# guangkun0818/speech2text

Measured on AMD Instinct MI355X. Metric: audio-seconds/sec (train step, zipformer pruned-RNN-T), higher is better.
Workload: dtype f32; 1 GPU; C3 zipformer pruned-RNN-T train step: chunk_size -1, 500 BPE, prune_range 5 (fbank+fwd+bwd+allreduce+ScaledAdam); accumulate_grad_batches=1, gemm_arith=bf16x2/3, per_gpu_batch=64, global_batch=64, labels_per_utt=50, parallelism=dp1

## Files before the change

include/s2t_mi355.h:

```cpp
#ifndef S2T_MI355_H_
#define S2T_MI355_H_

#ifdef __cplusplus
extern "C" {
#endif

int s2t_fbank_f32(const float* pcm, long pcm_stride, const long* num_samples, int batch,
                  const float* window400, const float* twiddle512, const int* mel_off,
                  const int* mel_k0, const float* mel_w, int nnz, int num_mel, float eps,
                  float scale_in, const float* cmvn_mean, const float* cmvn_istd, float* out,
                  int max_frames, long* out_frames, void* stream);

#define S2T_CTC_MAX_LABELS 1023
long s2t_ctc_workspace_floats(int B, int T, int Umax);
int s2t_ctc_loss_fwd_bwd(const float* logits, const long* targets, long tgt_stride,
                         const long* in_len, const long* tgt_len, int B, int T, int V, int Umax,
                         int blank, int zero_infinity, const float* grad_scale, float* workspace,
                         float* loss_per_utt, float* grad_logits, void* stream);

int s2t_fill_f32(float* p, long n, float v, void* stream);
int s2t_rnnt_row_exp(const float* x, long rows, int C, float* probs, float* rowmax, void* stream);
int s2t_rnnt_simple_pxpy(const float* am, const float* lm, const float* am_max,
                         const float* lm_max, const float* nrm, const long* symbols,
                         const long* boundary, int B, int S, int T, int C, int blank, float* px,
// ... 222 lines not shown
int s2t_specaug(float* feats, int B, int T, int F, const int* tspan, int nt, const int* fspan,
                int nf, void* stream);
int s2t_pad_rows(const float* packed, const long* offsets, int B, long Lmax, int D, float* out,
                 void* stream);

int s2t_linear_lt(int mode, const float* X, long ldx, const float* W, long ldw, const float* bias,
                  const float* C, long ldc, float beta, float* D, long ldd, int M, int N, int K,
                  void* workspace, long ws_bytes, void* stream);
int s2t_linear_lt_stats(int* plans, int* timed);
long s2t_linear_lt_own_calls(void);

int s2t_bypass_fwd(const float* orig, const float* src, const float* scale, long rows, int C,
                   float* out, void* stream);
int s2t_bypass_bwd(const float* orig, const float* src, const float* scale, const float* g,
                   long rows, int C, float* d_orig, float* d_src, float* d_scale, void* stream);
int s2t_bypass_bwd_acc(const float* orig, const float* src, const float* scale, const float* g,
                       const float* acc_in, long rows, int C, float* d_orig, float* d_src,
                       float* d_scale, void* stream);
int s2t_attn_delta_pairs(const float* W, const float* dW0, const float* dO1, const float* O1,
                         int dv1, const float* dO2, const float* O2, int dv2, int T, int B, int H,
                         float* delta, void* stream);
int s2t_bypass_fwd_mask(const float* orig, const float* src, const float* scale, const float* fm,
                        int B, long rows, int C, float* out, void* stream);
int s2t_bypass_bwd_mask(const float* orig, const float* src, const float* scale, const float* g,
                        const float* fm, int B, long rows, int C, float* d_orig, float* d_src,
                        float* d_scale, void* stream);
int s2t_downsample_fwd(const float* src, const float* w, int ds, int T, int B, int C, float* out,
                       void* stream);
int s2t_downsample_bwd(const float* src, const float* w, const float* g, int ds, int T, int B, int C,
                       float* d_src, float* dw, void* stream);
int s2t_downsample_fwd_bt(const float* src, const float* w, int ds, int T, int B, int C, float* out,
                          void* stream);
int s2t_downsample_bwd_bt(const float* src, const float* w, const float* g, int ds, int T, int B, int C,
                          float* d_src, float* dw, void* stream);
int s2t_bypass_up_fwd(const float* orig, const float* src, const float* scale, int up, int T, int B,
                      int C, float* out, void* stream);
int s2t_bypass_up_bwd(const float* orig, const float* src, const float* scale, const float* g, int up,
                      int T, int B, int C, float* d_orig, float* d_src, float* d_scale, void* stream);
typedef struct S2tCommit {
  const float* x;
  float* d;
  float* grad;
  float lo, hi;
  int limit;
  long n;
} S2tCommit;
int s2t_param_grad_commit_n(int n, const S2tCommit* items, void* stream);
int s2t_nonlin_gate_fwd(const float* u, int T, int B, int C, float* xs, void* stream);
int s2t_nonlin_out_fwd(const float* z, const float* u, int T, int B, int C, float* o, void* stream);
int s2t_nonlin_out_bwd(const float* g, const float* z, const float* u, int T, int B, int C, float* dz,
                       float* du, void* stream);
int s2t_nonlin_gate_bwd(const float* dxs, const float* u, int T, int B, int C, float* du,
                        void* stream);

int s2t_layernorm_fwd(const float* x, const float* y, float alpha, const float* gamma,
                      const float* beta, long rows, int C, float eps, float* xsum, float* out,
                      float* stats, void* stream);
typedef struct S2tLnFold {
  const float* partial;
  long rows;
  float* dgamma;
  float* dbeta;
} S2tLnFold;
long s2t_layernorm_bwd_partial_floats(long rows, int C);
int s2t_layernorm_bwd(const float* x, const float* stats, const float* gamma, const float* dy,
                      const float* resid, long rows, int C, float* dx, float* partial,
                      void* stream);
int s2t_layernorm_param_grad(int n, const S2tLnFold* items, int C, void* stream);
int s2t_silu_fwd(const float* h, long n, float* a, void* stream);
int s2t_silu_bwd(const float* h, const float* da, long n, float scale, float* dh, void* stream);
int s2t_dropout_add(const float* x, const float* y, long n, float alpha, float p,
                    unsigned long long seed, float* out, void* stream);
int s2t_silu_drop_fwd(const float* h, long n, float p, unsigned long long seed, float* a,
                      void* stream);
int s2t_silu_drop_bwd(const float* h, const float* da, long n, float scale, float p,
                      unsigned long long seed, float* dh, void* stream);
#define S2T_BN_PARTIALS 128
long s2t_bn_workspace_floats(int C);
int s2t_bn_silu_fwd(const float* x, const float* gamma, const float* beta, float eps,
                    float momentum, float* running_mean, float* running_var, long* num_batches,
                    long rows, int C, float* y, float* save_mean, float* save_rstd,
                    float* workspace, void* stream);
int s2t_bn_silu_apply(const float* x, const float* mean, const float* rstd, const float* gamma,
                      const float* beta, long rows, int C, float* y, void* stream);
int s2t_bn_silu_bwd(const float* x, const float* ds, const float* save_mean,
                    const float* save_rstd, const float* gamma, const float* beta, long rows, int C,
                    float* dx, float* dgamma, float* dbeta, float* workspace, void* stream);
int s2t_mhsa_fwd(const float* qkv, long ld, int qoff, int koff, int voff, const long* lens, int T,
                 int B, int H, int dh, float scale, float dropout_p, unsigned long seed, float* o,
                 long ldo, float* lse, void* stream);
int s2t_mhsa_bwd(const float* qkv, long ld, int qoff, int koff, int voff, const long* lens, int T,
                 int B, int H, int dh, float scale, float dropout_p, unsigned long seed,
                 const float* o, const float* d_o, long ldo, const float* lse, float* delta,
                 float* dqkv, void* stream);

long s2t_conv1_relu_workspace_floats(int C);
int s2t_conv1_relu_fwd(const float* x, const float* w, const float* bias, int B, int T, int F,
                       int C, float* out, void* stream);
int s2t_conv1_relu_wgrad(const float* x, const float* w, const float* bias, const float* d_out,
                         int B, int T, int F, int C, float* dw, float* db, float* workspace,
                         void* stream);

#define S2T_ADAM_MAX_GROUPS 8
typedef struct S2tAdamGroup {
  int chunk_hi;
  float lr, beta1, beta2, eps, weight_decay;
// ... 192 lines not shown
```

speech2text_amd/csrc/zip_glue.hip:

```cpp
#include "common.h"
#include "../../include/s2t_mi355.h"

namespace {

constexpr int RB = 64;

__global__ __launch_bounds__(256) void bypass_fwd_kernel(const float* __restrict__ orig,
                                                         const float* __restrict__ src,
                                                         const float* __restrict__ scale, long n4,
                                                         int C4, float* __restrict__ out) {
  const float4* o4 = reinterpret_cast<const float4*>(orig);
  const float4* s4 = reinterpret_cast<const float4*>(src);
  const float4* sc4 = reinterpret_cast<const float4*>(scale);
  float4* y4 = reinterpret_cast<float4*>(out);
  for (long i = (long)blockIdx.x * 256 + threadIdx.x; i < n4; i += (long)gridDim.x * 256) {
    const float4 a = o4[i], b = s4[i], k = sc4[i % C4];
    y4[i] = make_float4(fmaf(b.x - a.x, k.x, a.x), fmaf(b.y - a.y, k.y, a.y),
                        fmaf(b.z - a.z, k.z, a.z), fmaf(b.w - a.w, k.w, a.w));
  }
}

__global__ __launch_bounds__(256) void bypass_bwd_kernel(const float* __restrict__ orig,
                                                         const float* __restrict__ src,
                                                         const float* __restrict__ scale,
// ... 427 lines not shown
    const long t = tb / B;
    const float* row = u + tb * 3 * C;
    xs[((long)b * T + t) * C + c] = row[C + c] * tanhf(row[c]);
  }
}

__global__ __launch_bounds__(256) void nonlin_out_fwd_kernel(const float* __restrict__ z,
                                                             const float* __restrict__ u, int T,
                                                             int B, int C, float* __restrict__ o) {
  const long n = (long)T * B * C;
  for (long i = (long)blockIdx.x * 256 + threadIdx.x; i < n; i += (long)gridDim.x * 256) {
    const int c = (int)(i % C);
    const long tb = i / C;
    const int b = (int)(tb % B);
    const long t = tb / B;
    o[i] = z[((long)b * T + t) * C + c] * u[tb * 3 * C + 2 * C + c];
  }
}

__global__ __launch_bounds__(256) void nonlin_out_bwd_kernel(const float* __restrict__ g,
                                                             const float* __restrict__ z,
                                                             const float* __restrict__ u, int T,
                                                             int B, int C, float* __restrict__ dz,
                                                             float* __restrict__ du) {
  const long n = (long)T * B * C;
  for (long i = (long)blockIdx.x * 256 + threadIdx.x; i < n; i += (long)gridDim.x * 256) {
    const int c = (int)(i % C);
    const long tb = i / C;
    const int b = (int)(tb % B);
    const long t = tb / B;
    const long zi = ((long)b * T + t) * C + c;
    const float gv = g[i];
    dz[zi] = gv * u[tb * 3 * C + 2 * C + c];
    du[tb * 3 * C + 2 * C + c] = gv * z[zi];
  }
}

__global__ __launch_bounds__(256) void nonlin_gate_bwd_kernel(const float* __restrict__ dxs,
                                                              const float* __restrict__ u, int T,
                                                              int B, int C,
                                                              float* __restrict__ du) {
  const long n = (long)T * B * C;
  for (long i = (long)blockIdx.x * 256 + threadIdx.x; i < n; i += (long)gridDim.x * 256) {
    const int c = (int)(i % C);
    const long tb = i / C;
    const int b = (int)(tb % B);
    const long t = tb / B;
    const float d = dxs[((long)b * T + t) * C + c];
    const float* row = u + tb * 3 * C;
    const float th = tanhf(row[c]);
    du[tb * 3 * C + c] = d * row[C + c] * (1.f - th * th);
    du[tb * 3 * C + C + c] = d * th;
  }
}

inline unsigned grid1(long n) {
  long g = (n + 255) / 256;
  return (unsigned)(g > 4096 ? 4096 : (g < 1 ? 1 : g));
}

}

extern "C" int s2t_bypass_fwd(const float* orig, const float* src, const float* scale, long rows,
                              int C, float* out, void* stream) {
  if (rows <= 0) return 0;
  if (C <= 0 || (C & 3)) return -1;
  const long n4 = rows * C / 4;
  hipLaunchKernelGGL(bypass_fwd_kernel, dim3(grid1(n4)), dim3(256), 0, (hipStream_t)stream, orig,
                     src, scale, n4, C / 4, out);
  S2T_CHECK_LAUNCH();
  return 0;
}

extern "C" int s2t_bypass_bwd(const float* orig, const float* src, const float* scale,
                              const float* g, long rows, int C, float* d_orig, float* d_src,
                              float* d_scale, void* stream) {
  if (rows <= 0) return 0;
  if (C <= 0) return -1;
  hipLaunchKernelGGL(bypass_bwd_kernel, dim3((unsigned)((rows + RB - 1) / RB)), dim3(256), 0,
                     (hipStream_t)stream, orig, src, scale, g, rows, C, d_orig, d_src, d_scale);
  S2T_CHECK_LAUNCH();
  return 0;
}

extern "C" int s2t_bypass_bwd_acc(const float* orig, const float* src, const float* scale,
                                  const float* g, const float* acc_in, long rows, int C,
                                  float* d_orig, float* d_src, float* d_scale, void* stream) {
  if (rows <= 0) return 0;
  if (C <= 0 || !acc_in) return -1;
  hipLaunchKernelGGL(bypass_bwd_acc_kernel, dim3((unsigned)((rows + RB - 1) / RB)), dim3(256), 0,
                     (hipStream_t)stream, orig, src, scale, g, acc_in, rows, C, d_orig, d_src,
                     d_scale);
  S2T_CHECK_LAUNCH();
  return 0;
}

extern "C" int s2t_attn_delta_pairs(const float* W, const float* dW0, const float* dO1,
                                    const float* O1, int dv1, const float* dO2, const float* O2,
                                    int dv2, int T, int B, int H, float* delta, void* stream) {
  if (T <= 0 || B <= 0 || H <= 0) return 0;
  if (dv1 > 64 || dv2 > 64 || dv1 < 0 || dv2 < 0) return -1;
  const long rows = (long)H * B * T;
  hipLaunchKernelGGL(attn_delta_pairs_kernel, dim3((unsigned)((rows + 3) / 4)), dim3(256), 0,
                     (hipStream_t)stream, W, dW0, dO1, O1, dv1, dO2, O2, dv2, T, B, H, delta);
  S2T_CHECK_LAUNCH();
  return 0;
// ... 127 lines not shown
    nb = (nb + m - 1) / m * m;
#define BUP4(UP, IU)                                                                                          \
  hipLaunchKernelGGL((bypass_up_bwd4_kernel<UP, IU>), dim3((unsigned)nb), dim3(256), 0, (hipStream_t)stream,  \
                     reinterpret_cast<const float4*>(orig), reinterpret_cast<const float4*>(src),             \
                     reinterpret_cast<const float4*>(scale), reinterpret_cast<const float4*>(g), T, F, C4, n, \
                     reinterpret_cast<float4*>(d_orig), reinterpret_cast<float4*>(d_src), d_scale)
    if (up == 2) BUP4(2, 4);
    else if (up == 4) BUP4(4, 2);
    else BUP4(8, 1);
#undef BUP4
    S2T_CHECK_LAUNCH();
    return 0;
  }
  hipLaunchKernelGGL(bypass_up_bwd_kernel, dim3(Ts, (B + 15) / 16), dim3(256), 0,
                     (hipStream_t)stream, orig, src, scale, g, up, T, B, C, d_orig, d_src, d_scale);
  S2T_CHECK_LAUNCH();
  return 0;
}

extern "C" int s2t_nonlin_gate_fwd(const float* u, int T, int B, int C, float* xs, void* stream) {
  if (T <= 0 || B <= 0 || C <= 0) return 0;
  hipLaunchKernelGGL(nonlin_gate_fwd_kernel, dim3(grid1((long)T * B * C)), dim3(256), 0,
                     (hipStream_t)stream, u, T, B, C, xs);
  S2T_CHECK_LAUNCH();
  return 0;
}

extern "C" int s2t_nonlin_out_fwd(const float* z, const float* u, int T, int B, int C, float* o,
                                  void* stream) {
  if (T <= 0 || B <= 0 || C <= 0) return 0;
  hipLaunchKernelGGL(nonlin_out_fwd_kernel, dim3(grid1((long)T * B * C)), dim3(256), 0,
                     (hipStream_t)stream, z, u, T, B, C, o);
  S2T_CHECK_LAUNCH();
  return 0;
}

extern "C" int s2t_nonlin_out_bwd(const float* g, const float* z, const float* u, int T, int B,
                                  int C, float* dz, float* du, void* stream) {
  if (T <= 0 || B <= 0 || C <= 0) return 0;
  hipLaunchKernelGGL(nonlin_out_bwd_kernel, dim3(grid1((long)T * B * C)), dim3(256), 0,
                     (hipStream_t)stream, g, z, u, T, B, C, dz, du);
  S2T_CHECK_LAUNCH();
  return 0;
}

extern "C" int s2t_nonlin_gate_bwd(const float* dxs, const float* u, int T, int B, int C,
                                   float* du, void* stream) {
  if (T <= 0 || B <= 0 || C <= 0) return 0;
  hipLaunchKernelGGL(nonlin_gate_bwd_kernel, dim3(grid1((long)T * B * C)), dim3(256), 0,
                     (hipStream_t)stream, dxs, u, T, B, C, du);
  S2T_CHECK_LAUNCH();
  return 0;
}
```

speech2text_amd/csrc/zip_layer.hip:

```cpp
#include <hip/hip_runtime.h>

#include <cmath>
#include <cstdint>
#include <cstdio>
#include <cstring>
#include <atomic>
#include <functional>
#include <mutex>
#include <unordered_map>
#include <vector>

#include "../../include/s2t_mi355.h"
#include "common.h"

namespace {

constexpr int kMagic = 0x5a4c3532;
constexpr float kPenLimit = 25.0f;
constexpr int kMaxProb = 48;

thread_local char g_err[256] = "";

std::mutex g_mu;
float* g_pin = nullptr;
// ... 492 lines not shown
  sv.st.on = 0;
  if (fw) TRY(whiten_stats(c, sv.st, sv.y, c.d.D, R, c.d.D, m.wh.groups));
  *x_out = out;
  return 0;
}

int conv_fwd(Ctx& c, int i, int d0, const float* x_in, const float** x_out) {
  const S2tZlConv& m = c.d.cv[i];
  CvS& sv = c.s.cv[i];
  const bool fw = dec(c, d0 + 2);
  const long R = c.R;
  const int D = c.d.D, T = c.c.T, B = c.c.B;
  if (c.c.chunk_size >= 0 && !m.causal) return fail(-1, "conv module: chunk_size needs causal=True");
  sv.u = c.ar.alloc(R * 2 * D);
  Epi e;
  e.bias = m.in.b;
  TRY(lt_matmul(c, 0, x_in, D, R, m.in, e, sv.u));
  c.s.bst[6 + i] = c.s.bst[8 + i] = nullptr;
  if (dec(c, d0)) TRY(bal_stats_fwd(c, 6 + i, sv.u + D, 2 * D, R, D));
  sv.chunk = (c.c.chunk_size < 0 || c.c.chunk_size > T) ? T : c.c.chunk_size;
  sv.y = c.ar.alloc(R * D);
  sv.a = c.ar.alloc(R * D);
  RUN(s2t_zipconv_fwd_act(sv.u, 2 * D, D, c.c.k8, T, B, D, m.K, sv.chunk, m.wc, m.bc, m.wk, m.bk, m.scale, sv.y,
                          sv.a, 2, (void*)c.st));
  if (dec(c, d0 + 1)) TRY(bal_stats_fwd(c, 8 + i, sv.y, D, R, D, 4096, &m.bal2));
  sv.st.on = 0;
  if (fw) TRY(whiten_stats(c, sv.st, sv.y, D, R, D, m.wh.groups));
  float* out = c.ar.alloc(R * D);
  Epi e2;
  e2.bias = m.out.b;
  e2.resid2 = x_in;
  TRY(lt_matmul(c, 0, sv.a, D, R, m.out, e2, out));
  *x_out = out;
  return 0;
}

int na_fwd(Ctx& c, const float* x_in, const float** x_out) {
  const S2tZlNa& m = c.d.na;
  NaS& sv = c.s.na;
  const bool fw1 = dec(c, 8), fw2 = dec(c, 9), fp = dec(c, 10);
  const long R = c.R;
  const int D = c.d.D, T = c.c.T, B = c.c.B;
  const int C = m.in.N / 3;
  sv.C = C;
  sv.u = c.ar.alloc(R * 3 * C);
  Epi e;
  e.bias = m.in.b;
  TRY(lt_matmul(c, 0, x_in, D, R, m.in, e, sv.u));
  c.s.bst[10] = c.s.bst[11] = nullptr;
  if (dec(c, 7)) TRY(bal_stats_fwd(c, 11, sv.u, 3 * C, R, C));
  sv.xs = c.ar.alloc(R * C);
  RUN(s2t_nonlin_gate_fwd(sv.u, T, B, C, sv.xs, (void*)c.st));
  sv.z = c.ar.alloc(R * C);
  { const S2tGemmClass cls(0); TRY(bmm(c, 1, c.s.W, sv.xs, sv.z, B, T, C, T)); }
  sv.o = c.ar.alloc(R * C);
  RUN(s2t_nonlin_out_fwd(sv.z, sv.u, T, B, C, sv.o, (void*)c.st));
  sv.st1.on = 0;
  if (fw1) TRY(whiten_stats(c, sv.st1, sv.u + C, 3 * C, R, C, m.wh1.groups));
  float* out;
  TRY(out_proj(c, m.out, sv.o, R, x_in, fw2 || fp, &sv.y, &out));
  if (fp) TRY(bal_stats_fwd(c, 10, sv.y, D, R, D));
  sv.st2.on = 0;
  if (fw2) TRY(whiten_stats(c, sv.st2, sv.y, D, R, D, m.wh2.groups));
  *x_out = out;
  return 0;
}

int layer_fwd(Ctx& c) {
  const S2tZipLayerDesc& d = c.d;
  State& s = c.s;
  const int T = c.c.T, B = c.c.B, D = d.D, H = d.H, qd = d.qd, pd = d.pd;
  const long R = c.R;
  const int Dp = d.attn_in.N;
  s.magic = kMagic;
  s.T = T;
  s.B = B;
  s.nprob = 0;
  s.x[0] = c.c.x0;
  s.bal_fwd = 0;
  for (int i = 0; i < kBalSites; ++i) s.bst[i] = nullptr;
  s.qkp = c.ar.alloc(R * Dp);
  {
    Epi e;
    e.bias = d.attn_in.b;
    TRY(lt_matmul(c, 0, s.x[0], D, R, d.attn_in, e, s.qkp));
  }
  if (dec(c, 0)) TRY(bal_stats_fwd(c, 14, s.qkp + H * qd, Dp, R, H * qd));
  s.kst.on = 0;
  if (dec(c, 1)) TRY(whiten_stats(c, s.kst, s.qkp + H * qd, Dp, R, H * qd, d.wh_keys.groups));
  s.posp = nullptr;
  s.pos2 = c.c.pos;
  if (dec(c, 2)) {
    s.posp = c.ar.alloc((long)(2 * T - 1) * H * pd);
    Epi e;
    TRY(lt_matmul(c, 0, c.c.pos, d.pos_dim, 2 * T - 1, d.attn_pos, e, s.posp));
  }
  s.W = c.ar.alloc((long)H * B * T * T);
  s.pen_slot = nullptr;
  if (dec(c, 3)) {
    if (!c.dry) {
      s.pen_slot = pinned_slot();
      s.pen_ev = ring_event();
      if (!s.pen_slot || !s.pen_ev) return fail(-1, "penalty flag slot");
      *s.pen_slot = 0.f;
    }
    RUN(s2t_relpos_attn_fwd_flag(s.qkp, s.posp, c.c.k8, c.c.a8, T, B, H, qd, pd, s.W, kPenLimit, s.pen_slot,
                                 (void*)c.st));
    HIPRUN(hipEventRecord(s.pen_ev, c.st));
  } else {
// ... 123 lines not shown
      float* o = c.ar.alloc(R * D);
      TRY(balancer_bwd(c, m.bal2, sv.y, D, dy, D, R, D, o, D, -1.0f, c.s.bst[8 + i]));
      dy = o;
    }
  }
  float* du = c.ar.alloc(R * 2 * D);
  const long wsn = s2t_zipconv_bwd_workspace_floats(T, B, D, m.K);
  float* ws = c.ar.alloc(wsn);
  if (c.c.conv_w_side && c.side && !c.c.conv_fused) {
    RUN(s2t_zipconv_bwd_data(sv.u, 2 * D, D, c.c.k8, T, B, D, m.K, sv.chunk, m.wc, m.wk, m.bk, m.scale, dy, du,
                             (void*)c.st));
    if (!c.dry)
      TRY(side_run(c, [&c, &m, &sv, dy, ws, T, B, D]() -> int {
        RUN(s2t_zipconv_bwd_params(sv.u, 2 * D, D, c.c.k8, T, B, D, m.K, sv.chunk, m.wc, m.wk, m.bk, m.scale, dy,
                                   m.gwc, m.gbc, m.gwk, m.gbk, m.gscale, ws, (void*)c.side));
        return 0;
      }));
  } else {
    RUN(s2t_zipconv_bwd(sv.u, 2 * D, D, c.c.k8, T, B, D, m.K, sv.chunk, m.wc, m.wk, m.bk, m.scale, dy, du, m.gwc,
                        m.gbc, m.gwk, m.gbk, m.gscale, ws, (void*)c.st));
  }
  if (fb1) TRY(balancer_bwd(c, m.bal1, sv.u + D, 2 * D, du + D, 2 * D, R, D, du + D, 2 * D, -1.0f, c.s.bst[6 + i]));
  TRY(wgrad(c, m.in, du, 2 * D, x_in, D, R));
  float* gx = c.ar.alloc(R * D);
  Epi e;
  e.resid2 = g;
  TRY(lt_matmul(c, 1, du, 2 * D, R, m.in, e, gx));
  *g_out = gx;
  return 0;
}

int na_bwd(Ctx& c, const float* x_in, const float* g, const float** g_out) {
  const S2tZlNa& m = c.d.na;
  NaS& sv = c.s.na;
  const bool fb = dec(c, 7), fw1 = dec(c, 8), fw2 = dec(c, 9), fp = dec(c, 10);
  const long R = c.R;
  const int D = c.d.D, T = c.c.T, B = c.c.B, C = sv.C;
  const float* gy = g;
  if (fp) {
    float* o = c.ar.alloc(R * D);
    TRY(balancer_bwd(c, m.post, sv.y, D, gy, D, R, D, o, D, -1.0f, c.s.bst[10]));
    gy = o;
  }
  if (fw2) TRY(whiten_bwd(c, 3, m.wh2, sv.st2, sv.y, D, R, D, gy, &gy));
  TRY(wgrad(c, m.out, gy, D, sv.o, C, R));
  float* dout = c.ar.alloc(R * C);
  {
    Epi e;
    TRY(lt_matmul(c, 1, gy, D, R, m.out, e, dout));
  }
  float* dz = c.ar.alloc(R * C);
  float* du = c.ar.alloc(R * 3 * C);
  RUN(s2t_nonlin_out_bwd(dout, sv.z, sv.u, T, B, C, dz, du, (void*)c.st));
  float* dxs = c.ar.alloc(R * C);
  const S2tGemmClass cls_d(1);
  TRY(bmm(c, 2, c.s.W, dz, dxs, B, T, C, T));
  c.s.dW0 = c.ar.alloc((long)B * T * T);
  TRY(bmm(c, 0, dz, sv.xs, c.s.dW0, B, T, T, C));
  RUN(s2t_nonlin_gate_bwd(dxs, sv.u, T, B, C, du, (void*)c.st));
  if (fb) TRY(balancer_bwd(c, m.bal, sv.u, 3 * C, du, 3 * C, R, C, du, 3 * C, -1.0f, c.s.bst[11]));
  if (fw1) {
    float* gc = c.ar.alloc(R * C);
    TRY(copy2d(c, gc, C, du + C, 3 * C, C, R));
    const float* o;
    TRY(whiten_bwd(c, 2, m.wh1, sv.st1, sv.u + C, 3 * C, R, C, gc, &o));
    if (o != gc) TRY(copy2d(c, du + C, 3 * C, o, C, C, R));
  }
  TRY(wgrad(c, m.in, du, 3 * C, x_in, D, R));
  float* gx = c.ar.alloc(R * D);
  Epi e;
  e.resid2 = g;
  TRY(lt_matmul(c, 1, du, 3 * C, R, m.in, e, gx));
  *g_out = gx;
  return 0;
}

int layer_bwd(Ctx& c, int phase) {
  const S2tZipLayerDesc& d = c.d;
  State& s = c.s;
  const int T = c.c.T, B = c.c.B, D = d.D, H = d.H, qd = d.qd, pd = d.pd;
  const long R = c.R;
  const int Dp = d.attn_in.N;
  if (phase != 2) {
    s.nprob = 0;
    for (int i = 0; i < S2T_ZL_NWHITEN; ++i) s.wh_active[i] = -1;
    s.pen_active = 0;
    if (s.bal_fwd && !c.dry && !(g_bal_waited_on == (void*)c.st && s.bal_seq <= g_bal_waited)) {
      HIPRUN(hipStreamWaitEvent(c.st, s.bal_ev, 0));
      g_bal_waited_on = (void*)c.st;
      g_bal_waited = s.bal_seq;
    }
    if (dec(c, 3) && !c.dry) {
      if (hipEventSynchronize(s.pen_ev) != hipSuccess) return fail(-1, "penalty flag event");
      s.pen_active = *reinterpret_cast<volatile float*>(s.pen_slot) != 0.f;
    }
    const float* g = c.c.g;
    const float* x11 = s.x[11];
    if (dec(c, 30)) TRY(whiten_bwd(c, 10, d.wh_out, s.wst, x11, D, R, D, g, &g));
    if (dec(c, 29)) {
      float* o = c.ar.alloc(R * D);
      TRY(balancer_bwd(c, d.bal2, x11, D, g, D, R, D, o, D, -1.0f, s.bst[13]));
      g = o;
    }
    float* acc = c.c.layer_acc;
    float* d0 = c.ar.alloc(R * D);
    float* g9w = c.ar.alloc(R * D);
    RUN(s2t_norm_bypass_bwd(s.x[9], d.norm_bias.x, s.nscales, s.x[0], d.byp.x, g, s.fm_fused ? c.c.fm : nullptr, B,
                            R, D, g9w, d0, acc, acc + 2 * D, acc + 3 * D, (void*)c.st));
    const float* g9 = g9w;
    if (dec(c, 26)) {
      float* o = c.ar.alloc(R * D);
      TRY(balancer_bwd(c, d.bal1, s.x[9], D, g9, D, R, D, o, D, -1.0f, s.bst[12]));
// ... 184 lines not shown
```

speech2text_amd/zip_layer.py:

```python
import ctypes
import os

import torch

from . import _native as N
from . import flat
from . import zip_kernels as zk
from . import zip_native as zn
from .model.layer import scaling as S

_F32 = torch.float32
ENABLED = os.environ.get("S2T_LAYER_EXEC", "1") == "1"
CALLS = [0]
STATS = {"penalize": 0, "penalty_active": 0}
PEN_LIMIT, PEN_VALUE = 25.0, 1.0e-4


class _Plan:
    __slots__ = ("k_bal", "k_wh", "use_pos", "penalize", "ff1", "na", "sa1", "cv1", "ff2", "mid_lim", "sa2",
                 "cv2", "ff3", "bal1", "norm_lim", "byp_lim", "bal2", "wh_out")


def _bal(m):
    return S._rand() < float(m.prob)
# ... 242 lines not shown
    fb1, fb2, fw = dec
    sv = _Saved()
    D = x_in.shape[1]
    if chunk_size >= 0:
        assert m.causal, "Must initialize model with causal=True if you use chunk_size"
    sv.u = zk.lt_matmul(0, x_in, m.in_proj.weight, m.in_proj.bias)
    sv.cp = zk.conv_params(m.depthwise_conv, T, chunk_size)
    y, a = zk.zipconv_forward(sv.u.view(T, B, 2 * D), D, k8, *sv.cp, act=False)
    sv.y, sv.a = y.view(T * B, D), a.view(T * B, D)
    sv.st = zk.WhitenStats(sv.y, m.whiten.num_groups) if fw else None
    return zk.lt_matmul(0, sv.a, m.out_proj.weight, m.out_proj.bias, x_in), sv


def _conv_bwd(m, dec, sv, x_in, g, T, B, k8):
    fb1, fb2, fw = dec
    D = x_in.shape[1]
    W = m.out_proj.weight
    _wgrad(W, m.out_proj.bias, g, sv.a)
    if fb2 and not fw:
        dy = zk.lt_matmul(1, g, W, act_src=sv.y, act_kind="swoosh_r", bal=m.balancer2.cfg(2))
    else:
        dy = zk.lt_matmul(1, g, W, act_src=sv.y, act_kind="swoosh_r")
        if fw:
            dy = _whiten_bwd(m.whiten, sv.y, dy, sv.st)
        if fb2:
            dy = _balancer_bwd(m.balancer2, sv.y, dy)
    chunk, K, wc, bc, wk, bk, scale = sv.cp
    plist = (wc, bc, wk, bk, scale)
    grads = zk.direct_grads(plist)
    if grads is None:
        raise RuntimeError("zip_layer: conv-module parameters must live in a FlatStore")
    du = zk.zipconv_backward(sv.u.view(T, B, 2 * D), D, k8, chunk, K, wc, wk, bk, scale,
                             dy.view(T, B, D), grads).view(T * B, 2 * D)
    for p in plist:
        if p is not None:
            flat.grad_written(p)
    if fb1:
        _balancer_bwd(m.balancer1, sv.u[:, D:], du[:, D:], inplace=True)
    _wgrad(m.in_proj.weight, m.in_proj.bias, du, x_in)
    return zk.lt_matmul(1, du, m.in_proj.weight, None, g)


def _na_fwd(m, dec, x_in, W, T, B):
    fb, fw1, fw2, fp = dec
    sv = _Saved()
    L, st = N.lib(), N.stream()
    dev = x_in.device
    sv.u = zk.lt_matmul(0, x_in, m.in_proj.weight, m.in_proj.bias)
    C = sv.u.shape[1] // 3
    sv.xs = torch.empty((B, T, C), dtype=_F32, device=dev)
    N.PROF[0] and N.profile_note("s2t_nonlin_gate_fwd", 12.0 * T * B * C)
    N.check(L.s2t_nonlin_gate_fwd(N.fp(sv.u), T, B, C, N.fp(sv.xs), st), "nonlin_gate_fwd")
    sv.wm = W[0]
    with zk.gemm_class(zk.CLS_F):
        sv.z = zk.batched_matmul(1, sv.wm, sv.xs)
    sv.o = _e(T * B, C, dev)
    N.PROF[0] and N.profile_note("s2t_nonlin_out_fwd", 12.0 * T * B * C)
    N.check(L.s2t_nonlin_out_fwd(N.fp(sv.z), N.fp(sv.u), T, B, C, N.fp(sv.o), st),
            "nonlin_out_fwd")
    sv.st1 = zk.WhitenStats(sv.u[:, C:2 * C], m.whiten1.num_groups) if fw1 else None
    sv.y = sv.st2 = None
    if not (fw2 or fp):
        out = zk.lt_matmul(0, sv.o, m.out_proj.weight, m.out_proj.bias, x_in)
    else:
        sv.y, out = zk.lt_matmul(0, sv.o, m.out_proj.weight, m.out_proj.bias, act2="add", resid_b=x_in)
        if fw2:
            sv.st2 = zk.WhitenStats(sv.y, m.whiten2.num_groups)
    return out, sv


def _na_bwd(m, post, dec, sv, x_in, g, T, B):
    fb, fw1, fw2, fp = dec
    L, st = N.lib(), N.stream()
    gy = g
    if fp:
        gy = _balancer_bwd(post, sv.y, gy)
    if fw2:
        gy = _whiten_bwd(m.whiten2, sv.y, gy, sv.st2)
    _wgrad(m.out_proj.weight, m.out_proj.bias, gy, sv.o)
    do = zk.lt_matmul(1, gy, m.out_proj.weight)
    C = sv.u.shape[1] // 3
    dz = torch.empty_like(sv.z)
    du = torch.empty_like(sv.u)
    N.PROF[0] and N.profile_note("s2t_nonlin_out_bwd", 20.0 * T * B * C)
    N.check(L.s2t_nonlin_out_bwd(N.fp(do), N.fp(sv.z), N.fp(sv.u), T, B, C, N.fp(dz), N.fp(du), st),
            "nonlin_out_bwd")
    with zk.gemm_class(zk.CLS_D):
        dxs = zk.batched_matmul(2, sv.wm, dz)
        dW0 = zk.batched_matmul(0, dz, sv.xs)
    N.PROF[0] and N.profile_note("s2t_nonlin_gate_bwd", 20.0 * T * B * C)
    N.check(L.s2t_nonlin_gate_bwd(N.fp(dxs), N.fp(sv.u), T, B, C, N.fp(du), st), "nonlin_gate_bwd")
    if fb:
        _balancer_bwd(m.balancer, sv.u[:, :C], du[:, :C], inplace=True)
    if fw1:
        du[:, C:2 * C] = _whiten_bwd(m.whiten1, sv.u[:, C:2 * C], du[:, C:2 * C].contiguous(),
                                     sv.st1)
    _wgrad(m.in_proj.weight, m.in_proj.bias, du, x_in)
    return zk.lt_matmul(1, du, m.in_proj.weight, None, g), dW0


def _attn_bwd_penalized(s, qkp3, pairs, dW0, H, qd, pd):
    T, B, _ = qkp3.shape
    dW = None
    for dO, v, _, dv in pairs:
        t = torch.matmul(dO.view(T, B, H, dv).permute(2, 1, 0, 3), v.view(T, B, H, dv).permute(2, 1, 3, 0))
        dW = t if dW is None else dW.add_(t)
    dW[0] += dW0
    with torch.enable_grad():
        q_ = qkp3.detach().requires_grad_(True)
        p_ = None if s.posp is None else s.posp.detach().requires_grad_(True)
        w = zk.relpos_attention_weights(
            q_, p_, H, qd, pd, None if s.a8 is None else s.a8.bool(),
            None if s.k8 is None else s.k8.bool(),
            penalize=lambda sc: S.penalize_abs_values_gt(sc, limit=PEN_LIMIT, penalty=PEN_VALUE))
        ins = [q_] if p_ is None else [q_, p_]
        gs = torch.autograd.grad(w, ins, dW)
    return gs[0].contiguous(), (None if p_ is None else gs[1].contiguous())


class _LayerFn(torch.autograd.Function):
    @staticmethod
    def forward(ctx, src, pos_emb, layer, chunk_size, d, a8, k8, fm):
        T, B, D = src.shape
        R = T * B
        dev = src.device
        L, st = N.lib(), N.stream()
        x0 = src.contiguous().view(R, D)
        sa = layer.self_attn_weights
        H, qd, pd = sa.num_heads, sa.query_head_dim, sa.pos_head_dim
        s = _Saved()
        s.d, s.dims, s.x0, s.a8, s.k8 = d, (T, B, D, H, qd, pd), x0, a8, k8

        s.qkp = zk.lt_matmul(0, x0, sa.in_proj.weight, sa.in_proj.bias)
        s.kst = None
        if d.k_wh:
            s.kst = zk.WhitenStats(s.qkp[:, H * qd:2 * H * qd], sa.whiten_keys.num_groups)
        s.pos2 = s.posp = None
        if d.use_pos:
            s.pos2 = pos_emb.reshape(2 * T - 1, -1).contiguous().float()
            s.posp = zk.lt_matmul(0, s.pos2, sa.linear_pos.weight, None)
        W = torch.empty((H, B, T, T), dtype=_F32, device=dev)
        N.PROF[0] and N.profile_note("s2t_relpos_attn_fwd_flag" if d.penalize else "s2t_relpos_attn_fwd",
                                     4.0 * (s.qkp.numel() + W.numel()),
                                     2.0 * W.numel() * (qd + (pd if d.use_pos else 0)))
# ... 142 lines not shown
```

Measured before the change: 18430 audio-seconds/sec.

## Fuse attention-weight batched matmul with nonlin elementwise epilogues in fwd and bwd

Adds a custom MFMA bf16-split batched GEMM kernel for the NonlinAttention W0·xs product. Its epilogue writes z and the gated output o in the forward pass, and in the backward pass (W0ᵀ·dz) it writes the tanh-gated du halves directly. This removes the separate bmm plus elementwise kernels and the dxs intermediate buffer, saving launches and a round trip through global memory. In exchange, a hand-written GEMM with XCD tile swizzling may be slower than the library bmm for some shapes.

```diff
diff --git a/include/s2t_mi355.h b/include/s2t_mi355.h
--- a/include/s2t_mi355.h
+++ b/include/s2t_mi355.h
@@ -298,6 +298,10 @@
                        float* du, void* stream);
 int s2t_nonlin_gate_bwd(const float* dxs, const float* u, int T, int B, int C, float* du,
                         void* stream);
+int s2t_nonlin_w0x_fwd(const float* w0, const float* xs, const float* u, long ldu, int T, int B, int C,
+                       float* z, float* o, void* stream);
+int s2t_nonlin_w0t_bwd(const float* w0, const float* dz, const float* u, long ldu, int T, int B, int C,
+                       float* du, long lddu, void* stream);
 
 int s2t_layernorm_fwd(const float* x, const float* y, float alpha, const float* gamma,
                       const float* beta, long rows, int C, float eps, float* xsum, float* out,
diff --git a/speech2text_amd/csrc/zip_glue.hip b/speech2text_amd/csrc/zip_glue.hip
--- a/speech2text_amd/csrc/zip_glue.hip
+++ b/speech2text_amd/csrc/zip_glue.hip
@@ -503,6 +503,230 @@
     du[tb * 3 * C + c] = d * row[C + c] * (1.f - th * th);
     du[tb * 3 * C + C + c] = d * th;
   }
+}
+
+typedef float f32x16 __attribute__((ext_vector_type(16)));
+typedef float f32x2 __attribute__((ext_vector_type(2)));
+typedef __bf16 bf16x2 __attribute__((ext_vector_type(2)));
+typedef __bf16 bf16x8 __attribute__((ext_vector_type(8)));
+typedef unsigned u32x2_t __attribute__((ext_vector_type(2)));
+typedef unsigned u32x4_t __attribute__((ext_vector_type(4)));
+typedef const __attribute__((address_space(1))) float* gf32p;
+typedef __attribute__((address_space(1))) float* gf32w;
+
+__device__ __forceinline__ void na_split(float x0, float x1, bool np3, unsigned& p0, unsigned& p1,
+                                         unsigned& p2) {
+  f32x2 x = {x0, x1};
+  p0 = __builtin_bit_cast(unsigned, __builtin_convertvector(x, bf16x2));
+  f32x2 h = {__uint_as_float(p0 << 16), __uint_as_float(p0 & 0xFFFF0000u)};
+  x = x - h;
+  p1 = __builtin_bit_cast(unsigned, __builtin_convertvector(x, bf16x2));
+  p2 = 0u;
+  if (np3) {
+    f32x2 h1 = {__uint_as_float(p1 << 16), __uint_as_float(p1 & 0xFFFF0000u)};
+    x = x - h1;
+    p2 = __builtin_bit_cast(unsigned, __builtin_convertvector(x, bf16x2));
+  }
+}
+
+struct NaW0Args {
+  const float* W;
+  const float* Bm;
+  const float* u;
+  long ldu;
+  float* z;
+  float* o;
+  float* du;
+  long lddu;
+  int T, B, C;
+  int tiles_m, tiles_n;
+  int np;
+};
+
+template <int NP>
+__device__ __forceinline__ unsigned na_slot(int so, int kg) {
+  return (unsigned)(((((so >> 5) * 2 + (kg >> 1)) * NP) * 64 + (kg & 1) * 32 + (so & 31)) * 16);
+}
+
+constexpr unsigned NA_OOB = 0x7FFFFF00u;
+
+__device__ __forceinline__ float na_ld(__amdgpu_buffer_rsrc_t rs, unsigned off) {
+  return __uint_as_float(__builtin_amdgcn_raw_buffer_load_b32(rs, off, 0, 0));
+}
+
+template <bool TRANS, int NP>
+__global__ __launch_bounds__(256) void nonlin_w0_kernel(NaW0Args g) {
+  constexpr int BK = 32, IMG = 64 * BK * 2 * NP;
+  constexpr bool np3 = NP == 3;
+  __shared__ __attribute__((aligned(16))) unsigned char sA[IMG];
+  __shared__ __attribute__((aligned(16))) unsigned char sB[IMG];
+  const int total = g.tiles_m * g.tiles_n, per_xcd = (total + 7) / 8;
+  const int lin = (int)((blockIdx.x & 7) * per_xcd + (blockIdx.x >> 3));
+  if (lin >= total) return;
+  const int tm = lin / g.tiles_n, tn = lin - tm * g.tiles_n;
+  const int m0 = tm * 64, n0 = tn * 64;
+  const int b = blockIdx.y, T = g.T, C = g.C;
+  const __amdgpu_buffer_rsrc_t rsW = __builtin_amdgcn_make_buffer_rsrc(
+      const_cast<float*>(g.W) + (long)b * T * T, 0, T * T * 4, 0x00020000);
+  const __amdgpu_buffer_rsrc_t rsB = __builtin_amdgcn_make_buffer_rsrc(
+      const_cast<float*>(g.Bm) + (long)b * T * C, 0, T * C * 4, 0x00020000);
+  const int lane = threadIdx.x & 63, wave = threadIdx.x >> 6;
+  const int wm = (wave >> 1) * 32, wn = (wave & 1) * 32;
+
+  f32x16 acc;
+#pragma unroll
+  for (int r = 0; r < 16; ++r) acc[r] = 0.f;
+
+  const int so = threadIdx.x & 63, kg = threadIdx.x >> 6;
+  const unsigned sdst = na_slot<NP>(so, kg);
+  const int ar = threadIdx.x >> 3, kq = threadIdx.x & 7;
+  unsigned ob[8], oa[TRANS ? 8 : 2];
+#pragma unroll
+  for (int e = 0; e < 8; ++e) ob[e] = n0 + so < C ? (unsigned)(((8 * kg + e) * C + n0 + so) * 4) : NA_OOB;
+  if (TRANS) {
+#pragma unroll
+    for (int e = 0; e < 8; ++e) oa[e] = m0 + so < T ? (unsigned)(((8 * kg + e) * T + m0 + so) * 4) : NA_OOB;
+  } else {
+#pragma unroll
+    for (int i = 0; i < 2; ++i) oa[i] = (unsigned)(((m0 + ar + 32 * i) * T + 4 * kq) * 4);
+  }
+  const unsigned stepb = (unsigned)(BK * C * 4), stepa = TRANS ? (unsigned)(BK * T * 4) : (unsigned)(BK * 4);
+  float ra[8], rb[8];
+#define NA_LOAD()                                                                              \
+  {                                                                                            \
+    _Pragma("unroll") for (int e = 0; e < 8; ++e) {                                            \
+      rb[e] = na_ld(rsB, ob[e]);                                                               \
+      ob[e] += stepb;                                                                          \
+    }                                                                                          \
+    if (TRANS) {                                                                               \
+      _Pragma("unroll") for (int e = 0; e < 8; ++e) {                                          \
+        ra[e] = na_ld(rsW, oa[e]);                                                             \
+        oa[e] += stepa;                                                                        \
+      }                                                                                        \
+    } else {                                                                                   \
+      _Pragma("unroll") for (int i = 0; i < 2; ++i) {                                          \
+        const u32x4_t q_ = __builtin_amdgcn_raw_buffer_load_b128(rsW, oa[i], 0, 0);            \
+        ra[4 * i] = __uint_as_float(q_.x);                                                     \
+        ra[4 * i + 1] = __uint_as_float(q_.y);                                                 \
+        ra[4 * i + 2] = __uint_as_float(q_.z);                                                 \
+        ra[4 * i + 3] = __uint_as_float(q_.w);                                                 \
+        oa[i] += stepa;                                                                        \
+      }                                                                                        \
+    }                                                                                          \
+  }
+#define NA_STORE8(R, S)                                                                        \
+  {                                                                                            \
+    unsigned a_[3], b_[3], c_[3], d_[3];                                                       \
+    na_split(R[0], R[1], np3, a_[0], a_[1], a_[2]);                                            \
+    na_split(R[2], R[3], np3, b_[0], b_[1], b_[2]);                                            \
+    na_split(R[4], R[5], np3, c_[0], c_[1], c_[2]);                                            \
+    na_split(R[6], R[7], np3, d_[0], d_[1], d_[2]);                                            \
+    const u32x4_t q0_ = {a_[0], b_[0], c_[0], d_[0]}, q1_ = {a_[1], b_[1], c_[1], d_[1]},      \
+                  q2_ = {a_[2], b_[2], c_[2], d_[2]};                                          \
+    *reinterpret_cast<u32x4_t*>((S) + sdst) = q0_;                                             \
+    *reinterpret_cast<u32x4_t*>((S) + sdst + 1024) = q1_;                                      \
+    if (np3) *reinterpret_cast<u32x4_t*>((S) + sdst + 2048) = q2_;                             \
+  }
+  NA_LOAD()
+  for (int k0 = 0; k0 < T; k0 += BK) {
+    __syncthreads();
+    NA_STORE8(rb, sB)
+    if (TRANS) {
+      NA_STORE8(ra, sA)
+    } else {
+      if (k0 + BK > T) {
+#pragma unroll
+        for (int i = 0; i < 2; ++i)
+#pragma unroll
+          for (int j = 0; j < 4; ++j)
+            if (k0 + 4 * kq + j >= T) ra[4 * i + j] = 0.f;
+      }
+#pragma unroll
+      for (int i = 0; i < 2; ++i) {
+        unsigned a[3], c[3];
+        na_split(ra[4 * i], ra[4 * i + 1], np3, a[0], a[1], a[2]);
+        na_split(ra[4 * i + 2], ra[4 * i + 3], np3, c[0], c[1], c[2]);
+        const u32x2_t q0 = {a[0], c[0]}, q1 = {a[1], c[1]}, q2 = {a[2], c[2]};
+        unsigned char* d = sA + na_slot<NP>(ar + 32 * i, kq >> 1) + (kq & 1) * 8;
+        *reinterpret_cast<u32x2_t*>(d) = q0;
+        *reinterpret_cast<u32x2_t*>(d + 1024) = q1;
+        if (np3) *reinterpret_cast<u32x2_t*>(d + 2048) = q2;
+      }
+    }
+    __syncthreads();
+    if (k0 + BK < T) NA_LOAD()
+#pragma unroll
+    for (int s = 0; s < BK / 16; ++s) {
+      bf16x8 pa[NP], pb[NP];
+#pragma unroll
+      for (int p = 0; p < NP; ++p) {
+        pa[p] = *reinterpret_cast<const bf16x8*>(sA + (((wm >> 5) * 2 + s) * NP + p) * 1024 + lane * 16);
+        pb[p] = *reinterpret_cast<const bf16x8*>(sB + (((wn >> 5) * 2 + s) * NP + p) * 1024 + lane * 16);
+      }
+#define NA_TERM(PA, PB) acc = __builtin_amdgcn_mfma_f32_32x32x16_bf16(pa[PA], pb[PB], acc, 0, 0, 0);
+      if constexpr (np3) { NA_TERM(2, 0) NA_TERM(1, 1) NA_TERM(0, 2) }
+      NA_TERM(1, 0) NA_TERM(0, 1)
+      NA_TERM(0, 0)
+#undef NA_TERM
+    }
+  }
+#undef NA_LOAD
+#undef NA_STORE8
+  const int hi = lane >> 5, lo = lane & 31;
+  const int col = n0 + wn + lo, colc = min(col, C - 1);
+  const gf32p u = (gf32p)g.u;
+  if (!TRANS) {
+    float yv[16];
+#pragma unroll
+    for (int r = 0; r < 16; ++r) {
+      const int row = min(m0 + wm + (r & 3) + 8 * (r >> 2) + 4 * hi, T - 1);
+      yv[r] = u[((long)row * g.B + b) * g.ldu + 2 * C + colc];
+    }
+    const gf32w z = (gf32w)g.z, o = (gf32w)g.o;
+#pragma unroll
+    for (int r = 0; r < 16; ++r) {
+      const int row = m0 + wm + (r & 3) + 8 * (r >> 2) + 4 * hi;
+      if (row < T && col < C) {
+        z[((long)b * T + row) * C + col] = acc[r];
+        o[((long)row * g.B + b) * C + col] = acc[r] * yv[r];
+      }
+    }
+  } else {
+    float sv[16], xv[16];
+#pragma unroll
+    for (int r = 0; r < 16; ++r) {
+      const int row = min(m0 + wm + (r & 3) + 8 * (r >> 2) + 4 * hi, T - 1);
+      const long base = ((long)row * g.B + b) * g.ldu;
+      sv[r] = u[base + colc];
+      xv[r] = u[base + C + colc];
+    }
+    const gf32w du = (gf32w)g.du;
+#pragma unroll
+    for (int r = 0; r < 16; ++r) {
+      const int row = m0 + wm + (r & 3) + 8 * (r >> 2) + 4 * hi;
+      const float th = tanhf(sv[r]);
+      if (row < T && col < C) {
+        const long base = ((long)row * g.B + b) * g.lddu;
+        du[base + col] = acc[r] * xv[r] * (1.f - th * th);
+        du[base + C + col] = acc[r] * th;
+      }
+    }
+  }
+}
+
+template <bool TRANS>
+int nonlin_w0_launch(NaW0Args g, hipStream_t st) {
+  if ((long)g.T * g.T * 4 >= (long)NA_OOB || (long)g.T * g.C * 4 >= (long)NA_OOB) return -1;
+  g.tiles_m = (g.T + 63) / 64;
+  g.tiles_n = (g.C + 63) / 64;
+  g.np = s2t_gemm_arith();
+  const dim3 grid((unsigned)((g.tiles_m * g.tiles_n + 7) / 8 * 8), g.B);
+  if (g.np == 2)
+    hipLaunchKernelGGL((nonlin_w0_kernel<TRANS, 2>), grid, dim3(256), 0, st, g);
+  else
+    hipLaunchKernelGGL((nonlin_w0_kernel<TRANS, 3>), grid, dim3(256), 0, st, g);
+  S2T_CHECK_LAUNCH();
+  return 0;
 }
 
 inline unsigned grid1(long n) {
@@ -736,3 +960,19 @@
   S2T_CHECK_LAUNCH();
   return 0;
 }
+
+extern "C" int s2t_nonlin_w0x_fwd(const float* w0, const float* xs, const float* u, long ldu, int T,
+                                  int B, int C, float* z, float* o, void* stream) {
+  if (T <= 0 || B <= 0 || C <= 0) return 0;
+  if (B > 65535 || ldu < 3L * C || !w0 || !xs || !u || !z || !o) return -1;
+  NaW0Args g{w0, xs, u, ldu, z, o, nullptr, 0, T, B, C, 0, 0, 0};
+  return nonlin_w0_launch<false>(g, (hipStream_t)stream);
+}
+
+extern "C" int s2t_nonlin_w0t_bwd(const float* w0, const float* dz, const float* u, long ldu, int T,
+                                  int B, int C, float* du, long lddu, void* stream) {
+  if (T <= 0 || B <= 0 || C <= 0) return 0;
+  if (B > 65535 || ldu < 3L * C || lddu < 3L * C || !w0 || !dz || !u || !du) return -1;
+  NaW0Args g{w0, dz, u, ldu, nullptr, nullptr, du, lddu, T, B, C, 0, 0, 0};
+  return nonlin_w0_launch<true>(g, (hipStream_t)stream);
+}
diff --git a/speech2text_amd/csrc/zip_layer.hip b/speech2text_amd/csrc/zip_layer.hip
--- a/speech2text_amd/csrc/zip_layer.hip
+++ b/speech2text_amd/csrc/zip_layer.hip
@@ -568,9 +568,11 @@
   sv.xs = c.ar.alloc(R * C);
   RUN(s2t_nonlin_gate_fwd(sv.u, T, B, C, sv.xs, (void*)c.st));
   sv.z = c.ar.alloc(R * C);
-  { const S2tGemmClass cls(0); TRY(bmm(c, 1, c.s.W, sv.xs, sv.z, B, T, C, T)); }
   sv.o = c.ar.alloc(R * C);
-  RUN(s2t_nonlin_out_fwd(sv.z, sv.u, T, B, C, sv.o, (void*)c.st));
+  {
+    const S2tGemmClass cls(0);
+    RUN(s2t_nonlin_w0x_fwd(c.s.W, sv.xs, sv.u, 3L * C, T, B, C, sv.z, sv.o, (void*)c.st));
+  }
   sv.st1.on = 0;
   if (fw1) TRY(whiten_stats(c, sv.st1, sv.u + C, 3 * C, R, C, m.wh1.groups));
   float* out;
@@ -800,12 +802,10 @@
   float* dz = c.ar.alloc(R * C);
   float* du = c.ar.alloc(R * 3 * C);
   RUN(s2t_nonlin_out_bwd(dout, sv.z, sv.u, T, B, C, dz, du, (void*)c.st));
-  float* dxs = c.ar.alloc(R * C);
   const S2tGemmClass cls_d(1);
-  TRY(bmm(c, 2, c.s.W, dz, dxs, B, T, C, T));
+  RUN(s2t_nonlin_w0t_bwd(c.s.W, dz, sv.u, 3L * C, T, B, C, du, 3L * C, (void*)c.st));
   c.s.dW0 = c.ar.alloc((long)B * T * T);
   TRY(bmm(c, 0, dz, sv.xs, c.s.dW0, B, T, T, C));
-  RUN(s2t_nonlin_gate_bwd(dxs, sv.u, T, B, C, du, (void*)c.st));
   if (fb) TRY(balancer_bwd(c, m.bal, sv.u, 3 * C, du, 3 * C, R, C, du, 3 * C, -1.0f, c.s.bst[11]));
   if (fw1) {
     float* gc = c.ar.alloc(R * C);
diff --git a/speech2text_amd/zip_layer.py b/speech2text_amd/zip_layer.py
--- a/speech2text_amd/zip_layer.py
+++ b/speech2text_amd/zip_layer.py
@@ -318,12 +318,13 @@
     N.PROF[0] and N.profile_note("s2t_nonlin_gate_fwd", 12.0 * T * B * C)
     N.check(L.s2t_nonlin_gate_fwd(N.fp(sv.u), T, B, C, N.fp(sv.xs), st), "nonlin_gate_fwd")
     sv.wm = W[0]
+    sv.z = torch.empty((B, T, C), dtype=_F32, device=dev)
+    sv.o = _e(T * B, C, dev)
     with zk.gemm_class(zk.CLS_F):
-        sv.z = zk.batched_matmul(1, sv.wm, sv.xs)
-    sv.o = _e(T * B, C, dev)
-    N.PROF[0] and N.profile_note("s2t_nonlin_out_fwd", 12.0 * T * B * C)
-    N.check(L.s2t_nonlin_out_fwd(N.fp(sv.z), N.fp(sv.u), T, B, C, N.fp(sv.o), st),
-            "nonlin_out_fwd")
+        N.PROF[0] and N.profile_note("s2t_nonlin_w0x_fwd", 4.0 * B * T * T + 16.0 * T * B * C,
+                                     2.0 * B * T * T * C)
+        N.check(L.s2t_nonlin_w0x_fwd(N.fp(sv.wm), N.fp(sv.xs), N.fp(sv.u), 3 * C, T, B, C, N.fp(sv.z),
+                                     N.fp(sv.o), st), "nonlin_w0x_fwd")
     sv.st1 = zk.WhitenStats(sv.u[:, C:2 * C], m.whiten1.num_groups) if fw1 else None
     sv.y = sv.st2 = None
     if not (fw2 or fp):
@@ -352,10 +353,11 @@
     N.check(L.s2t_nonlin_out_bwd(N.fp(do), N.fp(sv.z), N.fp(sv.u), T, B, C, N.fp(dz), N.fp(du), st),
             "nonlin_out_bwd")
     with zk.gemm_class(zk.CLS_D):
-        dxs = zk.batched_matmul(2, sv.wm, dz)
+        N.PROF[0] and N.profile_note("s2t_nonlin_w0t_bwd", 4.0 * B * T * T + 20.0 * T * B * C,
+                                     2.0 * B * T * T * C)
+        N.check(L.s2t_nonlin_w0t_bwd(N.fp(sv.wm), N.fp(dz), N.fp(sv.u), 3 * C, T, B, C, N.fp(du), 3 * C, st),
+                "nonlin_w0t_bwd")
         dW0 = zk.batched_matmul(0, dz, sv.xs)
-    N.PROF[0] and N.profile_note("s2t_nonlin_gate_bwd", 20.0 * T * B * C)
-    N.check(L.s2t_nonlin_gate_bwd(N.fp(dxs), N.fp(sv.u), T, B, C, N.fp(du), st), "nonlin_gate_bwd")
     if fb:
         _balancer_bwd(m.balancer, sv.u[:, :C], du[:, :C], inplace=True)
     if fw1:
```

Result: no change. 18340 audio-seconds/sec, median of 3 (-0.5%).
